# bioinformatics-ua/polus

Measured on AMD Instinct MI355X. Metric: train samples/sec BioBERT-base NER seq256, higher is better.
Workload: dtype bf16; 1 GPU; BERT-base (L=12,H=768,A=12,I=3072,V=28996) token classification C=4, seq_len=256, 64 samples/GPU, AdamW lr 5e-5 wd 0.01 warm-up 10%, dropout 0.1 (hidden + attention) (BASELINE.json configs[2] per-GPU shape), random-init weights; global_batch=64, seq_len=256, parallelism=dp1, grad_allreduce=none

## Files before the change

### polus_amd/csrc/common.h

```cpp
#pragma once
#include <hip/hip_runtime.h>
#include <stdint.h>
#include <stdio.h>
#include <string.h>
#include <math.h>

#include "../../include/polus_hip.h"

typedef __bf16 bf16_t;
typedef __bf16 bf16x8 __attribute__((ext_vector_type(8)));
typedef __bf16 bf16x4 __attribute__((ext_vector_type(4)));
typedef short s16x4 __attribute__((ext_vector_type(4)));
typedef float f32x4 __attribute__((ext_vector_type(4)));

void polus_set_error(const char* fmt, ...);
#define POLUS_FAIL(...) do { polus_set_error(__VA_ARGS__); return POLUS_ERR_INVALID; } while (0)
#define POLUS_REQUIRE(cond, ...) do { if (!(cond)) { polus_set_error(__VA_ARGS__); return POLUS_ERR_INVALID; } } while (0)
#define POLUS_CHECK_LAUNCH(name) do { hipError_t e__ = hipGetLastError(); \
    if (e__ != hipSuccess) { polus_set_error("%s: launch failed: %s", name, hipGetErrorString(e__)); return POLUS_ERR_HIP; } } while (0)
#define POLUS_HIP(call) do { hipError_t e__ = (call); \
    if (e__ != hipSuccess) { polus_set_error("%s failed: %s", #call, hipGetErrorString(e__)); return POLUS_ERR_HIP; } } while (0)

template <auto Kern, typename... A>
int polus_launch_lds(const char* who, dim3 grid, dim3 block, size_t lds_max, size_t lds, hipStream_t st, const A&... args) {
    static bool attr_done = false;
    if (!attr_done) {
        POLUS_HIP(hipFuncSetAttribute(reinterpret_cast<const void*>(Kern), hipFuncAttributeMaxDynamicSharedMemorySize, (int)lds_max));
        attr_done = true;
    }
    hipLaunchKernelGGL(Kern, grid, block, lds, st, args...);
    POLUS_CHECK_LAUNCH(who);
    return POLUS_OK;
}

static inline size_t polus_dtype_size(int dt) { return dt == POLUS_BF16 ? 2 : 4; }
static inline bool polus_aligned16(const void* p) { return (((uintptr_t)p) & 15) == 0; }

struct PolusCfg {
    int gemm_pp;
    int gemm_v1;
    int dw_ungrouped;
    int dw_fused_reduce;
    int ln_bwd_blocks;
    int ln_fin_single;
    int gemm_ring128;
    int gemm_auto_split;
    int ln_halfwave;
    int gemm_order;
    int gemm_persist;
    int reserve_cus;
    int attn_bwd_kres;
    int attn_debug;
    int dw_streamk;
    int dw_sk_cus;
    int dw_sk_delta;
    int attn_fused;
};
const PolusCfg& polus_cfg();
int polus_num_cus();
int polus_reserved_cus();

struct PolusDyn { uint32_t salt; float lr, lr_t; uint32_t pad; };
const PolusDyn* polus_dyn();
__device__ __forceinline__ uint32_t polus_eff_seed(uint32_t seed, const PolusDyn* dyn) {
    if (!dyn) return seed;
    uint32_t x = seed + dyn->salt;
    x ^= x >> 15;
    return x * 0x2C1B3C6Du;
}

template <typename T> __device__ __forceinline__ float to_f(T x);
template <> __device__ __forceinline__ float to_f<float>(float x) { return x; }
template <> __device__ __forceinline__ float to_f<bf16_t>(bf16_t x) { return (float)x; }
template <typename T> __device__ __forceinline__ T from_f(float x);
template <> __device__ __forceinline__ float from_f<float>(float x) { return x; }
template <> __device__ __forceinline__ bf16_t from_f<bf16_t>(float x) { return (bf16_t)x; }

template <typename T> __device__ __forceinline__ void load4(const T* p, float (&v)[4]);
template <> __device__ __forceinline__ void load4<float>(const float* p, float (&v)[4]) {
    float4 t = *reinterpret_cast<const float4*>(p); v[0] = t.x; v[1] = t.y; v[2] = t.z; v[3] = t.w;
}
template <> __device__ __forceinline__ void load4<bf16_t>(const bf16_t* p, float (&v)[4]) {
    bf16x4 t = *reinterpret_cast<const bf16x4*>(p);
    v[0] = (float)t[0]; v[1] = (float)t[1]; v[2] = (float)t[2]; v[3] = (float)t[3];
}
template <typename T> __device__ __forceinline__ void store4(T* p, const float (&v)[4]);
template <> __device__ __forceinline__ void store4<float>(float* p, const float (&v)[4]) {
    *reinterpret_cast<float4*>(p) = make_float4(v[0], v[1], v[2], v[3]);
}
template <> __device__ __forceinline__ void store4<bf16_t>(bf16_t* p, const float (&v)[4]) {
    bf16x4 t; t[0] = (bf16_t)v[0]; t[1] = (bf16_t)v[1]; t[2] = (bf16_t)v[2]; t[3] = (bf16_t)v[3];
    *reinterpret_cast<bf16x4*>(p) = t;
}

__device__ __forceinline__ float erf_fast(float x) {
    const float ax = fabsf(x);
    const float t = __frcp_rn(1.0f + 0.3275911f * ax);
    float poly = 1.061405429f;
    poly = poly * t - 1.453152027f;
    poly = poly * t + 1.421413741f;
    poly = poly * t - 0.284496736f;
    poly = poly * t + 0.254829592f;
    const float r = 1.0f - poly * t * __expf(-ax * ax);
    return copysignf(r, x);
}
__device__ __forceinline__ float gelu_f(float x) { return 0.5f * x * (1.0f + erf_fast(x * 0.70710678118654752f)); }
__device__ __forceinline__ float gelu_grad_f(float x) {
    float cdf = 0.5f * (1.0f + erf_fast(x * 0.70710678118654752f));
    float pdf = 0.3989422804014327f * __expf(-0.5f * x * x);
    return cdf + x * pdf;
}
__device__ __forceinline__ float swish_f(float x) { return x / (1.0f + __expf(-x)); }
__device__ __forceinline__ float swish_grad_f(float x) {
    float s = 1.0f / (1.0f + __expf(-x));
    return s * (1.0f + x * (1.0f - s));
}
typedef float f32x2_t __attribute__((ext_vector_type(2)));
__device__ __forceinline__ f32x2_t gelu_poly2(f32x2_t x, const float (&c)[11]) {
    f32x2_t xc = {__builtin_amdgcn_fmed3f(x[0], -4.5f, 4.5f), __builtin_amdgcn_fmed3f(x[1], -4.5f, 4.5f)};
    f32x2_t s = xc * xc;
    f32x2_t u = __builtin_elementwise_fma(s, (f32x2_t){2.0f / 20.25f, 2.0f / 20.25f}, (f32x2_t){-1.0f, -1.0f});
    f32x2_t r = {c[10], c[10]};
#pragma unroll
    for (int k = 9; k >= 0; --k) r = __builtin_elementwise_fma(r, u, (f32x2_t){c[k], c[k]});
    return __builtin_elementwise_fma(xc, r, (f32x2_t){0.5f, 0.5f});
}
__device__ __forceinline__ f32x2_t gelu_cdf2(f32x2_t x) {
    const float q[11] = {1.569049305e-01f, -7.719386095e-02f, 5.470119065e-02f, -4.010921159e-02f, 2.828393083e-02f,
                         -1.902094059e-02f, 1.143922652e-02f, -5.251548121e-03f, 2.716277400e-03f, -2.340015935e-03f,
                         9.806926012e-04f};
    return gelu_poly2(x, q);
}
__device__ __forceinline__ f32x2_t gelu_grad2(f32x2_t x) {
    const float w[11] = {1.594289755e-01f, -9.003904569e-02f, 8.714168751e-02f, -9.350841452e-02f, 9.645831298e-02f,
                         -9.557466143e-02f, 7.437658385e-02f, -3.356380937e-02f, 2.252388123e-02f, -3.068672777e-02f,
                         1.457471506e-02f};
    return gelu_poly2(x, w);
}
// ... 131 lines not shown
```

### polus_amd/csrc/norm.hip

```cpp
#include "common.h"

namespace {

constexpr int MAXC = 8;
constexpr int WAVES = 16;
constexpr int LN_THREADS = 64 * WAVES;
constexpr int MAX_PARTIAL_BLOCKS = 256;

__device__ __forceinline__ int n_chunks(int H) { return (H + 255) >> 8; }

template <typename T, int NC>
__device__ __forceinline__ void load_row(const T* row, int H, int lane, float (&v)[NC][4]) {
#pragma unroll
    for (int c = 0; c < NC; ++c) {
        int col = (lane + 64 * c) * 4;
        if (col < H) load4<T>(row + col, v[c]);
        else { v[c][0] = v[c][1] = v[c][2] = v[c][3] = 0.f; }
    }
}

template <int NC>
__device__ __forceinline__ void load_feat(const float* __restrict__ p, int H, int lane, float (&v)[NC][4]) {
#pragma unroll
    for (int c = 0; c < NC; ++c) {
// ... 192 lines not shown
        if (col < H) {
#pragma unroll
            for (int e = 0; e < 4; ++e) {
                xh[c][e] = (xv[c][e] - mu) * rs;
                dxh[c][e] = dy[c][e] * gv[c][e];
                s1 += dxh[c][e];
                s2 += dxh[c][e] * xh[c][e];
                acc.dg[c][e] += dy[c][e] * xh[c][e];
                acc.db[c][e] += dy[c][e];
            }
        } else {
#pragma unroll
            for (int e = 0; e < 4; ++e) xh[c][e] = dxh[c][e] = 0.f;
        }
    }
    s1 = wave_sum(s1) / (float)H;
    s2 = wave_sum(s2) / (float)H;
#pragma unroll
    for (int c = 0; c < NC; ++c) {
        int col = (lane + 64 * c) * 4;
        if (col < H) {
            float o[4], om[4];
#pragma unroll
            for (int e = 0; e < 4; ++e) { o[e] = (dxh[c][e] - s1 - xh[c][e] * s2) * rs; om[e] = o[e]; }
            if (out_drop.thresh) polus_dropout_run<4>(om, out_drop.seed, rowbase + col, out_drop.thresh, out_drop.inv, true);
            if (want_bias) {
#pragma unroll
                for (int e = 0; e < 4; ++e) acc.dbias[c][e] += om[e];
            }
            store4<TDX>(dxrow + col, o);
            if (dxm_row) store4<TDX>(dxm_row + col, om);
        }
    }
}

constexpr int BWD_WAVES = 4, BWD_MAX_BLOCKS = 1024, FIN_GROUP = 128;
template <typename T, int NC>
__global__ __launch_bounds__(64 * BWD_WAVES) void ln_bwd_kernel(const T* __restrict__ dy, const T* __restrict__ x,
                                                     const float* __restrict__ gamma, const float* __restrict__ mean,
                                                     const float* __restrict__ rstd, T* __restrict__ dx,
                                                     float* __restrict__ partial, int rows, int H, int want_bias,
                                                     T* __restrict__ dxm, DropArgs drop) {
    if (drop.thresh) drop.seed = polus_eff_seed(drop.seed, drop.dyn);
    extern __shared__ __attribute__((aligned(16))) unsigned char smem_raw[];
    float* lds = reinterpret_cast<float*>(smem_raw);
    const int lane = threadIdx.x & 63, wid = threadIdx.x >> 6;
    ColAcc<NC> acc;
    colacc_zero(acc);
    float gv[NC][4];
    load_feat<NC>(gamma, H, lane, gv);
    for (int row = blockIdx.x * BWD_WAVES + wid; row < rows; row += gridDim.x * BWD_WAVES) {
        float xv[NC][4];
        load_row<T, NC>(x + (long)row * H, H, lane, xv);
        ln_bwd_row<T, T, NC>(xv, dy + (long)row * H, gv, dx + (long)row * H, H, lane, mean[row], rstd[row], acc, want_bias,
                             dxm ? dxm + (long)row * H : nullptr, drop, DropArgs{0, 0, 1.f}, (unsigned)row * (unsigned)H);
    }
    colacc_flush_par<NC, BWD_WAVES>(acc, lds, partial, H, lane, wid, want_bias);
}

__global__ __launch_bounds__(1024) void colsum_finalize_kernel(const float* __restrict__ partial, int P, int pstride,
                                                               int ncols, int seg, float* out0, float* out1,
                                                               float* out2, int accumulate, int pgroup = 0) {
    __shared__ float red[16][64];
    const int cx = threadIdx.x & 63, gy = threadIdx.x >> 6;
    const int col = blockIdx.x * 64 + cx;
    float s = 0.f;
    if (pgroup > 0) {
        const int p0 = blockIdx.y * pgroup;
        partial += (long)p0 * pstride;
        P = min(pgroup, P - p0);
        out0 += (long)blockIdx.y * ncols;
    }
    if (col < ncols) {
#pragma unroll 8
        for (int p = gy; p < P; p += 16) s += partial[(long)p * pstride + col];
    }
    red[gy][cx] = s;
    __syncthreads();
    if (gy == 0 && col < ncols) {
        float t = 0.f;
#pragma unroll
        for (int k = 0; k < 16; ++k) t += red[k][cx];
        int which = col / seg, c = col % seg;
        float* out = which == 0 ? out0 : which == 1 ? out1 : out2;
        if (out) out[c] = accumulate ? out[c] + t : t;
    }
}

template <int NC>
__global__ __launch_bounds__(64 * BWD_WAVES) void ln_bwd_hw_kernel(const bf16_t* __restrict__ dy, const bf16_t* __restrict__ x,
                                                                    const float* __restrict__ gamma, const float* __restrict__ mean,
                                                                    const float* __restrict__ rstd, bf16_t* __restrict__ dx,
                                                                    float* __restrict__ partial, int rows, int H, int want_bias,
                                                                    bf16_t* __restrict__ dxm, DropArgs drop) {
    if (drop.thresh) drop.seed = polus_eff_seed(drop.seed, drop.dyn);
    extern __shared__ __attribute__((aligned(16))) unsigned char smem_raw[];
    float* lds = reinterpret_cast<float*>(smem_raw);
    const int lane = threadIdx.x & 63, wid = threadIdx.x >> 6, half = lane >> 5, hl = lane & 31;
    float gv[NC][8], adg[NC][8], adb[NC][8], abias[NC][8];
#pragma unroll
    for (int c = 0; c < NC; ++c) {
        const int col = (hl + 32 * c) * 8;
        load4<float>(gamma + col, *reinterpret_cast<float(*)[4]>(&gv[c][0])); load4<float>(gamma + col + 4, *reinterpret_cast<float(*)[4]>(&gv[c][4]));
#pragma unroll
        for (int e = 0; e < 8; ++e) adg[c][e] = adb[c][e] = abias[c][e] = 0.f;
    }
    const float invH = 1.0f / (float)H;
    for (int row = (blockIdx.x * BWD_WAVES + wid) * 2 + half; row < rows; row += gridDim.x * BWD_WAVES * 2) {
        const float mu = mean[row], rs = rstd[row];
        float xh[NC][8], dxh[NC][8];
        float s1 = 0.f, s2 = 0.f;
#pragma unroll
        for (int c = 0; c < NC; ++c) {
            const long off = (long)row * H + (hl + 32 * c) * 8;
            const bf16x8v tx = *reinterpret_cast<const bf16x8v*>(x + off);
            const bf16x8v td = *reinterpret_cast<const bf16x8v*>(dy + off);
#pragma unroll
            for (int e = 0; e < 8; ++e) {
                const float d = (float)td[e];
                xh[c][e] = ((float)tx[e] - mu) * rs;
                dxh[c][e] = d * gv[c][e];
                s1 += dxh[c][e];
                s2 += dxh[c][e] * xh[c][e];
                adg[c][e] += d * xh[c][e];
                adb[c][e] += d;
            }
        }
        s1 = half_sum(s1) * invH;
        s2 = half_sum(s2) * invH;
#pragma unroll
        for (int c = 0; c < NC; ++c) {
            const int col = (hl + 32 * c) * 8;
            float o[8], om[8];
#pragma unroll
            for (int e = 0; e < 8; ++e) { o[e] = (dxh[c][e] - s1 - xh[c][e] * s2) * rs; om[e] = o[e]; }
            if (drop.thresh) polus_dropout_run<8>(om, drop.seed, (unsigned)row * (unsigned)H + col, drop.thresh, drop.inv, true);
            if (want_bias) {
#pragma unroll
                for (int e = 0; e < 8; ++e) abias[c][e] += om[e];
            }
            bf16x8v t;
#pragma unroll
            for (int e = 0; e < 8; ++e) t[e] = (bf16_t)o[e];
            *reinterpret_cast<bf16x8v*>(dx + (long)row * H + col) = t;
            if (dxm) {
#pragma unroll
                for (int e = 0; e < 8; ++e) t[e] = (bf16_t)om[e];
                *reinterpret_cast<bf16x8v*>(dxm + (long)row * H + col) = t;
            }
        }
    }
    float* mine = lds + (long)wid * 3 * H;
#pragma unroll
    for (int c = 0; c < NC; ++c) {
        const int col = (hl + 32 * c) * 8;
#pragma unroll
        for (int e = 0; e < 8; ++e) {
            adg[c][e] += __shfl_xor(adg[c][e], 32, 64);
            adb[c][e] += __shfl_xor(adb[c][e], 32, 64);
            abias[c][e] += __shfl_xor(abias[c][e], 32, 64);
        }
        if (half == 0) {
            *reinterpret_cast<float4*>(mine + col) = make_float4(adg[c][0], adg[c][1], adg[c][2], adg[c][3]);
            *reinterpret_cast<float4*>(mine + col + 4) = make_float4(adg[c][4], adg[c][5], adg[c][6], adg[c][7]);
            *reinterpret_cast<float4*>(mine + H + col) = make_float4(adb[c][0], adb[c][1], adb[c][2], adb[c][3]);
            *reinterpret_cast<float4*>(mine + H + col + 4) = make_float4(adb[c][4], adb[c][5], adb[c][6], adb[c][7]);
            *reinterpret_cast<float4*>(mine + 2 * H + col) = make_float4(abias[c][0], abias[c][1], abias[c][2], abias[c][3]);
// ... 176 lines not shown
#pragma unroll
                for (int k = 0; k < 4; ++k)
                    row[j][c][k] = (valid && c * 256 + k * 64 + lane < H) ? src[c * 256 + k * 64] : 0.f;
        }
#pragma unroll
        for (int t = 0; t < SC_RUN; ++t) {
            const int id = __shfl(mine, t, 64);
            const unsigned same = (unsigned)__ballot(mine == id);
            if (id < 0 || (same & ((1u << t) - 1u))) continue;
            float* dst = gword + (long)id * H + lane;
#pragma unroll
            for (int c = 0; c < NC; ++c)
#pragma unroll
                for (int k = 0; k < 4; ++k) {
                    float acc = row[t][c][k];
#pragma unroll
                    for (int j = t + 1; j < SC_RUN; ++j)
                        if ((same >> j) & 1u) acc += row[j][c][k];
                    if (c * 256 + k * 64 + lane < H) atomicAdd(dst + c * 256 + k * 64, acc);
                }
        }
    }
}
__global__ __launch_bounds__(LN_THREADS) void embed_scatter_atomic_wide_kernel(const float* __restrict__ de, const int32_t* __restrict__ ids,
                                                                        float* __restrict__ gword, int rows, int H, int vocab) {
    const int lane = threadIdx.x & 63, wid = threadIdx.x >> 6;
    for (int row = blockIdx.x * WAVES + wid; row < rows; row += gridDim.x * WAVES) {
        int id = ids[row]; id = id < 0 ? 0 : (id >= vocab ? vocab - 1 : id);
        const float* src = de + (long)row * H;
        float* dst = gword + (long)id * H;
        for (int col = lane; col < H; col += 64) atomicAdd(dst + col, src[col]);
    }
}

__global__ __launch_bounds__(LN_THREADS) void embed_scatter_owner_kernel(const float* __restrict__ de, const int32_t* __restrict__ ids,
                                                                  float* __restrict__ gword, int rows, int H, int vocab) {
    const int lane = threadIdx.x & 63, wid = threadIdx.x >> 6;
    for (int row = blockIdx.x * WAVES + wid; row < rows; row += gridDim.x * WAVES) {
        auto clampid = [vocab](int v) { return v < 0 ? 0 : (v >= vocab ? vocab - 1 : v); };
        const int cid = clampid(ids[row]);
        bool dup = false;
        for (int j0 = 0; j0 < row && !dup; j0 += 64) {
            int j = j0 + lane;
            bool hit = (j < row) && (clampid(ids[j]) == cid);
            dup = __any(hit);
        }
        if (dup) continue;
        float* dst = gword + (long)cid * H;
        for (int c0 = 0; c0 < H; c0 += 64 * 4) {
            int col = c0 + lane * 4;
            float a[4] = {0.f, 0.f, 0.f, 0.f};
            for (int j0 = row; j0 < rows; j0 += 64) {
                int j = j0 + lane;
                unsigned long long m = __ballot((j < rows) && (clampid(ids[j]) == cid));
                while (m) {
                    int b = __ffsll((long long)m) - 1;
                    m &= m - 1;
                    if (col < H) {
                        float v[4];
                        load4<float>(de + (long)(j0 + b) * H + col, v);
#pragma unroll
                        for (int e = 0; e < 4; ++e) a[e] += v[e];
                    }
                }
            }
            if (col < H) {
                float o[4];
                load4<float>(dst + col, o);
#pragma unroll
                for (int e = 0; e < 4; ++e) o[e] += a[e];
                store4<float>(dst + col, o);
            }
        }
    }
}

__global__ __launch_bounds__(256) void embed_pos_grad_kernel(const float* __restrict__ de, float* __restrict__ gpos,
                                                             int B, int S, int H, int accumulate) {
    long idx = (long)blockIdx.x * blockDim.x + threadIdx.x;
    if (idx >= (long)S * H) return;
    float s = 0.f;
    for (int b = 0; b < B; ++b) s += de[(long)b * S * H + idx];
    gpos[idx] = accumulate ? gpos[idx] + s : s;
}

}

extern "C" size_t polus_layernorm_bwd_workspace_bytes(int rows, int H) {
    int b = ln_bwd_blocks(rows), b2 = ln_blocks(rows);
    if (b2 > b) b = b2;
    int groups = (b + FIN_GROUP - 1) / FIN_GROUP;
    return ((size_t)b + groups) * 3 * (size_t)H * sizeof(float);
}

extern "C" int polus_layernorm_fwd(int dtype, const void* x, const float* gamma, const float* beta,
                                   void* y, float* mean, float* rstd, int rows, int H, float eps, void* stream) {
    POLUS_REQUIRE(x && gamma && beta && y && mean && rstd, "polus_layernorm_fwd: null pointer");
    POLUS_REQUIRE(rows > 0 && H > 0 && H % 4 == 0 && H <= 256 * MAXC, "polus_layernorm_fwd: H=%d must be a multiple of 4, <= %d", H, 256 * MAXC);
    POLUS_REQUIRE(polus_aligned16(x) && polus_aligned16(y) && polus_aligned16(gamma) && polus_aligned16(beta),
                  "polus_layernorm_fwd: pointers must be 16-byte aligned");
    hipStream_t st = static_cast<hipStream_t>(stream);
    int blocks = (rows + WAVES - 1) / WAVES;
    if (blocks > 4096) blocks = 4096;
    if (dtype == POLUS_BF16 && H % 256 == 0 && H <= 1024 && rows % 2 == 0 && polus_cfg().ln_halfwave) {
        const int fw = 4;
        int hb = (rows / 2 + fw - 1) / fw;
        if (hb > 16384) hb = 16384;
        const int LN_THREADS_HW = 64 * fw;
        if (H == 256) hipLaunchKernelGGL(ln_fwd_hw_kernel<1>, dim3(hb), dim3(LN_THREADS_HW), 0, st, (const bf16_t*)x, gamma, beta, (bf16_t*)y, mean, rstd, rows, H, eps);
        else if (H == 512) hipLaunchKernelGGL(ln_fwd_hw_kernel<2>, dim3(hb), dim3(LN_THREADS_HW), 0, st, (const bf16_t*)x, gamma, beta, (bf16_t*)y, mean, rstd, rows, H, eps);
        else if (H == 768) hipLaunchKernelGGL(ln_fwd_hw_kernel<3>, dim3(hb), dim3(LN_THREADS_HW), 0, st, (const bf16_t*)x, gamma, beta, (bf16_t*)y, mean, rstd, rows, H, eps);
        else hipLaunchKernelGGL(ln_fwd_hw_kernel<4>, dim3(hb), dim3(LN_THREADS_HW), 0, st, (const bf16_t*)x, gamma, beta, (bf16_t*)y, mean, rstd, rows, H, eps);
    } else if (dtype == POLUS_BF16)
        POLUS_NC_DISPATCH(H, bf16_t, ln_fwd_kernel, dim3(blocks), dim3(LN_THREADS), 0, st, (const bf16_t*)x, gamma, beta, (bf16_t*)y, mean, rstd, rows, H, eps);
    else if (dtype == POLUS_F32)
        POLUS_NC_DISPATCH(H, float, ln_fwd_kernel, dim3(blocks), dim3(LN_THREADS), 0, st, (const float*)x, gamma, beta, (float*)y, mean, rstd, rows, H, eps);
    else POLUS_FAIL("polus_layernorm_fwd: bad dtype");
    POLUS_CHECK_LAUNCH("polus_layernorm_fwd");
    return POLUS_OK;
}

extern "C" int polus_layernorm_bwd(int dtype, const void* dy, const void* x, const float* gamma,
                                   const float* mean, const float* rstd, void* dx,
                                   float* dgamma, float* dbeta, float* dbias, int accumulate,
                                   int rows, int H, void* dx_masked, float drop_p, uint32_t seed,
                                   void* workspace, size_t workspace_bytes, void* stream) {
    const bool defer = !dgamma && !dbeta;
    POLUS_REQUIRE(dy && x && gamma && mean && rstd && dx && (defer || (dgamma && dbeta)), "polus_layernorm_bwd: null pointer");
    POLUS_REQUIRE(drop_p >= 0.f && drop_p < 1.f && (long)rows * H < (1LL << 32), "polus_layernorm_bwd: bad dropout arguments");
    POLUS_REQUIRE(!(drop_p > 0.f) || dx_masked, "polus_layernorm_bwd: dropout needs dx_masked");
    DropArgs drop{drop_p > 0.f ? polus_drop_thresh(drop_p) : 0u, seed, 1.0f / (1.0f - drop_p), polus_dyn()};
    POLUS_REQUIRE(rows > 0 && H > 0 && H % 4 == 0 && H <= 256 * MAXC, "polus_layernorm_bwd: bad H=%d", H);
    POLUS_REQUIRE(polus_aligned16(x) && polus_aligned16(dy) && polus_aligned16(dx) && polus_aligned16(gamma),
                  "polus_layernorm_bwd: pointers must be 16-byte aligned");
    size_t need = polus_layernorm_bwd_workspace_bytes(rows, H);
    if (!workspace || workspace_bytes < need) { polus_set_error("polus_layernorm_bwd: workspace %zu < %zu", workspace_bytes, need); return POLUS_ERR_WORKSPACE; }
    hipStream_t st = static_cast<hipStream_t>(stream);
    int blocks = ln_bwd_blocks(rows);
    float* partial = static_cast<float*>(workspace);
    size_t lds = (size_t)BWD_WAVES * 3 * (size_t)H * sizeof(float);
    int wb = dbias ? 1 : 0;
    if (dtype == POLUS_BF16 && H % 256 == 0 && H <= 1024 && rows % 2 == 0 && polus_cfg().ln_halfwave && polus_aligned16(dx_masked)) {
#define POLUS_LN_BWD_HW(NCV) hipLaunchKernelGGL(ln_bwd_hw_kernel<NCV>, dim3(blocks), dim3(64 * BWD_WAVES), lds, st, (const bf16_t*)dy, (const bf16_t*)x, gamma, mean, rstd, (bf16_t*)dx, partial, rows, H, wb, (bf16_t*)dx_masked, drop)
        if (H == 256) POLUS_LN_BWD_HW(1); else if (H == 512) POLUS_LN_BWD_HW(2); else if (H == 768) POLUS_LN_BWD_HW(3); else POLUS_LN_BWD_HW(4);
#undef POLUS_LN_BWD_HW
    } else if (dtype == POLUS_BF16)
        POLUS_NC_DISPATCH(H, bf16_t, ln_bwd_kernel, dim3(blocks), dim3(64 * BWD_WAVES), lds, st, (const bf16_t*)dy, (const bf16_t*)x, gamma, mean, rstd, (bf16_t*)dx, partial, rows, H, wb, (bf16_t*)dx_masked, drop);
    else if (dtype == POLUS_F32)
        POLUS_NC_DISPATCH(H, float, ln_bwd_kernel, dim3(blocks), dim3(64 * BWD_WAVES), lds, st, (const float*)dy, (const float*)x, gamma, mean, rstd, (float*)dx, partial, rows, H, wb, (float*)dx_masked, drop);
    else POLUS_FAIL("polus_layernorm_bwd: bad dtype");
    POLUS_CHECK_LAUNCH("polus_layernorm_bwd");
    if (defer) return POLUS_OK;
    int ncols = (wb ? 3 : 2) * H;
    if (blocks > polus_cfg().ln_fin_single) {
        int groups = (blocks + FIN_GROUP - 1) / FIN_GROUP;
        float* part2 = partial + (size_t)blocks * 3 * H;
        hipLaunchKernelGGL(colsum_finalize_kernel, dim3((ncols + 63) / 64, groups), dim3(1024), 0, st,
                           partial, blocks, 3 * H, ncols, ncols, part2, (float*)nullptr, (float*)nullptr, 0, FIN_GROUP);
        POLUS_CHECK_LAUNCH("polus_layernorm_bwd(finalize 1)");
        hipLaunchKernelGGL(colsum_finalize_kernel, dim3((ncols + 63) / 64), dim3(1024), 0, st,
                           part2, groups, ncols, ncols, H, dgamma, dbeta, dbias, accumulate, 0);
    } else {
        hipLaunchKernelGGL(colsum_finalize_kernel, dim3((ncols + 63) / 64), dim3(1024), 0, st,
                           partial, blocks, 3 * H, ncols, H, dgamma, dbeta, dbias, accumulate, 0);
    }
    POLUS_CHECK_LAUNCH("polus_layernorm_bwd(finalize)");
    return POLUS_OK;
}

extern "C" int polus_layernorm_bwd_finalize(void* workspace, size_t workspace_bytes, int rows, int H, float* dgamma, float* dbeta,
                                            float* dbias, int accumulate, void* stream) {
    POLUS_REQUIRE(workspace && dgamma && dbeta && rows > 0 && H > 0 && H % 4 == 0, "polus_layernorm_bwd_finalize: bad arguments");
    size_t need = polus_layernorm_bwd_workspace_bytes(rows, H);
    if (workspace_bytes < need) { polus_set_error("polus_layernorm_bwd_finalize: workspace %zu < %zu", workspace_bytes, need); return POLUS_ERR_WORKSPACE; }
    hipStream_t st = static_cast<hipStream_t>(stream);
    const int blocks = ln_bwd_blocks(rows);
    float* partial = static_cast<float*>(workspace);
    const int ncols = (dbias ? 3 : 2) * H;
    if (blocks > polus_cfg().ln_fin_single) {
        int groups = (blocks + FIN_GROUP - 1) / FIN_GROUP;
        float* part2 = partial + (size_t)blocks * 3 * H;
        hipLaunchKernelGGL(colsum_finalize_kernel, dim3((ncols + 63) / 64, groups), dim3(1024), 0, st,
                           partial, blocks, 3 * H, ncols, ncols, part2, (float*)nullptr, (float*)nullptr, 0, FIN_GROUP);
        POLUS_CHECK_LAUNCH("polus_layernorm_bwd_finalize(1)");
        hipLaunchKernelGGL(colsum_finalize_kernel, dim3((ncols + 63) / 64), dim3(1024), 0, st,
                           part2, groups, ncols, ncols, H, dgamma, dbeta, dbias, accumulate, 0);
    } else {
        hipLaunchKernelGGL(colsum_finalize_kernel, dim3((ncols + 63) / 64), dim3(1024), 0, st,
                           partial, blocks, 3 * H, ncols, H, dgamma, dbeta, dbias, accumulate, 0);
    }
    POLUS_CHECK_LAUNCH("polus_layernorm_bwd_finalize");
    return POLUS_OK;
}

extern "C" size_t polus_colsum_workspace_bytes(int rows, int cols) {
    int chunks = (rows + 63) / 64;
    if (chunks > 256) chunks = 256;
    if (chunks < 1) chunks = 1;
    return (size_t)chunks * (size_t)cols * sizeof(float);
}

extern "C" int polus_colsum(int dtype, const void* x, long ldx, int rows, int cols, float* out, int accumulate,
                            void* workspace, size_t workspace_bytes, void* stream) {
    POLUS_REQUIRE(x && out && rows > 0 && cols > 0 && ldx >= cols, "polus_colsum: bad arguments");
    POLUS_REQUIRE(dtype == POLUS_F32 || dtype == POLUS_BF16, "polus_colsum: bad dtype");
    return colsum_launch(dtype, x, ldx, rows, cols, out, accumulate, nullptr, 0, workspace, workspace_bytes,
                         static_cast<hipStream_t>(stream));
}

extern "C" size_t polus_embed_bwd_workspace_bytes(int B, int S, int H) {
    size_t rows = (size_t)B * S;
    size_t de = rows * H * sizeof(float);
    size_t part = polus_layernorm_bwd_workspace_bytes((int)rows, H);
    size_t cs = polus_colsum_workspace_bytes((int)rows, H);
    return de + (part > cs ? part : cs) + 256;
}

extern "C" int polus_embed_ln_fwd(int dtype, const int32_t* ids, const int32_t* type_ids,
                                  const float* word, const float* pos, const float* type,
                                  const float* gamma, const float* beta, void* y, float* mean, float* rstd,
                                  int B, int S, int H, int vocab, int max_pos, int type_vocab, float eps,
                                  float drop_p, uint32_t seed, void* stream) {
    POLUS_REQUIRE(ids && word && pos && type && gamma && beta && y && mean && rstd, "polus_embed_ln_fwd: null pointer");
    POLUS_REQUIRE(drop_p >= 0.f && drop_p < 1.f, "polus_embed_ln_fwd: bad drop_p");
    const unsigned dthresh = drop_p > 0.f ? polus_drop_thresh(drop_p) : 0u;
    const float dinv = 1.0f / (1.0f - drop_p);
    POLUS_REQUIRE(B > 0 && S > 0 && S <= max_pos, "polus_embed_ln_fwd: S=%d exceeds max_position_embeddings=%d", S, max_pos);
    POLUS_REQUIRE(H % 4 == 0 && H <= 256 * MAXC && vocab > 0 && type_vocab > 0, "polus_embed_ln_fwd: bad H=%d", H);
    POLUS_REQUIRE(polus_aligned16(word) && polus_aligned16(pos) && polus_aligned16(type) && polus_aligned16(y) &&
                  polus_aligned16(gamma) && polus_aligned16(beta), "polus_embed_ln_fwd: pointers must be 16-byte aligned");
    hipStream_t st = static_cast<hipStream_t>(stream);
    int rows = B * S, blocks = (rows + WAVES - 1) / WAVES;
    if (blocks > 4096) blocks = 4096;
    if (dtype == POLUS_BF16)
        POLUS_NC_DISPATCH(H, bf16_t, embed_fwd_kernel, dim3(blocks), dim3(LN_THREADS), 0, st, ids, type_ids, word, pos, type, gamma, beta, (bf16_t*)y, mean, rstd, B, S, H, vocab, type_vocab, eps, dthresh, seed, dinv, polus_dyn());
    else if (dtype == POLUS_F32)
        POLUS_NC_DISPATCH(H, float, embed_fwd_kernel, dim3(blocks), dim3(LN_THREADS), 0, st, ids, type_ids, word, pos, type, gamma, beta, (float*)y, mean, rstd, B, S, H, vocab, type_vocab, eps, dthresh, seed, dinv, polus_dyn());
    else POLUS_FAIL("polus_embed_ln_fwd: bad dtype");
    POLUS_CHECK_LAUNCH("polus_embed_ln_fwd");
    return POLUS_OK;
}

extern "C" int polus_embed_ln_bwd(int dtype, const void* dy, const int32_t* ids, const int32_t* type_ids,
                                  const float* word, const float* pos, const float* type, const float* gamma,
                                  const float* mean, const float* rstd,
                                  float* gword, float* gpos, float* gtype, float* ggamma, float* gbeta,
                                  int accumulate, int deterministic,
                                  int B, int S, int H, int vocab, int max_pos, int type_vocab,
                                  float drop_p, uint32_t seed,
                                  void* workspace, size_t workspace_bytes, void* stream) {
    DropArgs in_drop{drop_p > 0.f ? polus_drop_thresh(drop_p) : 0u, seed, 1.0f / (1.0f - drop_p), polus_dyn()};
    POLUS_REQUIRE(dy && ids && word && pos && type && gamma && mean && rstd && gword && gpos && gtype && ggamma && gbeta,
                  "polus_embed_ln_bwd: null pointer");
    POLUS_REQUIRE(B > 0 && S > 0 && S <= max_pos && H % 4 == 0 && H <= 256 * MAXC, "polus_embed_ln_bwd: bad shape");
    POLUS_REQUIRE(polus_aligned16(dy) && polus_aligned16(gword) && polus_aligned16(workspace),
                  "polus_embed_ln_bwd: pointers must be 16-byte aligned");
    size_t need = polus_embed_bwd_workspace_bytes(B, S, H);
    if (!workspace || workspace_bytes < need) { polus_set_error("polus_embed_ln_bwd: workspace %zu < %zu", workspace_bytes, need); return POLUS_ERR_WORKSPACE; }
    hipStream_t st = static_cast<hipStream_t>(stream);
    const int rows = B * S;
    float* de = static_cast<float*>(workspace);
    size_t de_bytes = ((size_t)rows * H * sizeof(float) + 255) / 256 * 256;
    float* partial = reinterpret_cast<float*>(static_cast<unsigned char*>(workspace) + de_bytes);
    size_t partial_bytes = workspace_bytes - de_bytes;
    int blocks = ln_blocks(rows);
    size_t lds = 3 * (size_t)H * sizeof(float);
    if (dtype == POLUS_BF16)
        POLUS_NC_DISPATCH(H, bf16_t, embed_bwd_ln_kernel, dim3(blocks), dim3(LN_THREADS), lds, st, (const bf16_t*)dy, ids, type_ids, word, pos, type, gamma, mean, rstd, de, partial, B, S, H, vocab, type_vocab, in_drop);
    else if (dtype == POLUS_F32)
        POLUS_NC_DISPATCH(H, float, embed_bwd_ln_kernel, dim3(blocks), dim3(LN_THREADS), lds, st, (const float*)dy, ids, type_ids, word, pos, type, gamma, mean, rstd, de, partial, B, S, H, vocab, type_vocab, in_drop);
    else POLUS_FAIL("polus_embed_ln_bwd: bad dtype");
    POLUS_CHECK_LAUNCH("polus_embed_ln_bwd(ln)");
    hipLaunchKernelGGL(colsum_finalize_kernel, dim3((2 * H + 63) / 64), dim3(1024), 0, st,
                       partial, blocks, 3 * H, 2 * H, H, ggamma, gbeta, (float*)nullptr, accumulate);
    POLUS_CHECK_LAUNCH("polus_embed_ln_bwd(finalize)");

    if (!accumulate) {
        POLUS_HIP(hipMemsetAsync(gword, 0, (size_t)vocab * H * sizeof(float), st));
        POLUS_HIP(hipMemsetAsync(gpos, 0, (size_t)max_pos * H * sizeof(float), st));
    }
    int sblocks = (rows + WAVES - 1) / WAVES;
    if (sblocks > 4096) sblocks = 4096;
    if (deterministic)
        hipLaunchKernelGGL(embed_scatter_owner_kernel, dim3(sblocks), dim3(LN_THREADS), 0, st, de, ids, gword, rows, H, vocab);
    else
    {
        const dim3 g(min((rows + SC_RUN * SC_WAVES - 1) / (SC_RUN * SC_WAVES), 4096)), b(64 * SC_WAVES);
        if (H <= 256) hipLaunchKernelGGL(embed_scatter_atomic_kernel<1>, g, b, 0, st, de, ids, gword, rows, H, vocab);
        else if (H <= 512) hipLaunchKernelGGL(embed_scatter_atomic_kernel<2>, g, b, 0, st, de, ids, gword, rows, H, vocab);
        else if (H <= 768) hipLaunchKernelGGL(embed_scatter_atomic_kernel<3>, g, b, 0, st, de, ids, gword, rows, H, vocab);
        else if (H <= 1024) hipLaunchKernelGGL(embed_scatter_atomic_kernel<4>, g, b, 0, st, de, ids, gword, rows, H, vocab);
        else hipLaunchKernelGGL(embed_scatter_atomic_wide_kernel, dim3(sblocks), dim3(LN_THREADS), 0, st, de, ids, gword, rows, H, vocab);
    }
    POLUS_CHECK_LAUNCH("polus_embed_ln_bwd(scatter)");
    hipLaunchKernelGGL(embed_pos_grad_kernel, dim3(((long)S * H + 255) / 256), dim3(256), 0, st, de, gpos, B, S, H, accumulate);
    POLUS_CHECK_LAUNCH("polus_embed_ln_bwd(pos)");
    for (int t = 0; t < type_vocab; ++t) {
        if (type_ids) {
            int rc = colsum_launch(POLUS_F32, de, H, rows, H, gtype + (long)t * H, accumulate, type_ids, t, partial, partial_bytes, st);
            if (rc != POLUS_OK) return rc;
        } else if (t == 0) {
            int rc = colsum_launch(POLUS_F32, de, H, rows, H, gtype, accumulate, nullptr, 0, partial, partial_bytes, st);
            if (rc != POLUS_OK) return rc;
        } else if (!accumulate) {
            POLUS_HIP(hipMemsetAsync(gtype + (long)t * H, 0, (size_t)H * sizeof(float), st));
        }
    }
    return POLUS_OK;
}
```

### polus_amd/csrc/runtime.hip

```cpp
#include "common.h"
#include <stdarg.h>

static thread_local char g_err[512] = "";

void polus_set_error(const char* fmt, ...) {
    va_list ap;
    va_start(ap, fmt);
    vsnprintf(g_err, sizeof(g_err), fmt, ap);
    va_end(ap);
}

extern "C" const char* polus_last_error(void) { return g_err; }

static PolusCfg g_cfg;
static bool g_cfg_ready = false;
static int env_int(const char* name, int dflt) {
    const char* e = getenv(name);
    return (e && *e) ? atoi(e) : dflt;
}
static void read_cfg() {
    g_cfg.gemm_pp = env_int("POLUS_GEMM_PP", 0);
    g_cfg.gemm_v1 = getenv("POLUS_GEMM_V1") != nullptr;
    g_cfg.dw_ungrouped = getenv("POLUS_DW_UNGROUPED") != nullptr;
    g_cfg.gemm_order = env_int("POLUS_GEMM_ORDER", 4);
    g_cfg.reserve_cus = env_int("POLUS_GEMM_RESERVE_CUS", 0);
    g_cfg.gemm_persist = env_int("POLUS_GEMM_PERSIST", 1);
    g_cfg.dw_fused_reduce = env_int("POLUS_DW_FUSED_REDUCE", 1);
    g_cfg.attn_fused = env_int("POLUS_ATTN_FUSED", 1);
    g_cfg.attn_bwd_kres = env_int("POLUS_ATTN_BWD_KRES", 1);
    g_cfg.attn_debug = env_int("POLUS_ATTN_DEBUG", 0);
    g_cfg.ln_halfwave = env_int("POLUS_LN_HALFWAVE", 1);
    g_cfg.gemm_auto_split = env_int("POLUS_GEMM_AUTO_SPLIT", 1);
    g_cfg.gemm_ring128 = env_int("POLUS_GEMM_RING128", 0);
    g_cfg.ln_bwd_blocks = env_int("POLUS_LN_BWD_BLOCKS", 512);
    g_cfg.ln_fin_single = env_int("POLUS_LN_FIN_SINGLE", 512);
    g_cfg.dw_streamk = env_int("POLUS_DW_STREAMK", 0);
    g_cfg.dw_sk_delta = env_int("POLUS_DW_SK_DELTA", 2);
    g_cfg.dw_sk_cus = env_int("POLUS_DW_SK_CUS", 0);
    g_cfg_ready = true;
}
const PolusCfg& polus_cfg() {
    if (!g_cfg_ready) read_cfg();
    return g_cfg;
}
extern "C" int polus_reload_env(void) { read_cfg(); return POLUS_OK; }

int polus_num_cus() {
    static int n = 0;
    if (!n) {
        int dev = 0; hipDeviceProp_t prop;
        if (hipGetDevice(&dev) == hipSuccess && hipGetDeviceProperties(&prop, dev) == hipSuccess) n = prop.multiProcessorCount;
        if (n <= 0) n = 256;
    }
    return n;
}
static int g_reserve_on = 1;
extern "C" int polus_set_reserve_active(int on) { g_reserve_on = on != 0; return POLUS_OK; }
int polus_reserved_cus() { return g_reserve_on ? polus_cfg().reserve_cus : 0; }

static const PolusDyn* g_dyn = nullptr;
const PolusDyn* polus_dyn() { return g_dyn; }
extern "C" int polus_set_dynamic_params(const void* dev_block16) {
    POLUS_REQUIRE(dev_block16 == nullptr || polus_aligned16(dev_block16), "polus_set_dynamic_params: the block must be 16-byte aligned");
    g_dyn = static_cast<const PolusDyn*>(dev_block16);
    return POLUS_OK;
}
extern "C" int polus_abi_version(void) { return POLUS_ABI_VERSION; }

extern "C" int polus_device_info(int* n_cu, int* lds_bytes_per_cu, char* arch, int arch_len) {
    int dev = 0;
    POLUS_HIP(hipGetDevice(&dev));
    hipDeviceProp_t prop;
    POLUS_HIP(hipGetDeviceProperties(&prop, dev));
    if (n_cu) *n_cu = prop.multiProcessorCount;
    if (lds_bytes_per_cu) *lds_bytes_per_cu = (int)prop.maxSharedMemoryPerMultiProcessor;
    if (arch && arch_len > 0) {
        strncpy(arch, prop.gcnArchName, arch_len - 1);
        arch[arch_len - 1] = 0;
    }
    return POLUS_OK;
}

namespace {

template <typename S, typename D>
__global__ void cast_kernel(const S* __restrict__ src, D* __restrict__ dst, int64_t n) {
    int64_t i4 = ((int64_t)blockIdx.x * blockDim.x + threadIdx.x) * 4;
    const int64_t stride = (int64_t)gridDim.x * blockDim.x * 4;
    for (; i4 < n; i4 += stride) {
        if (i4 + 4 <= n) {
            float v[4];
            load4<S>(src + i4, v);
            store4<D>(dst + i4, v);
        } else {
            for (int64_t j = i4; j < n; ++j) dst[j] = from_f<D>(to_f<S>(src[j]));
        }
    }
}

__global__ void scale_kernel(float* __restrict__ x, float a, int64_t n) {
    int64_t i4 = ((int64_t)blockIdx.x * blockDim.x + threadIdx.x) * 4;
    const int64_t stride = (int64_t)gridDim.x * blockDim.x * 4;
    for (; i4 < n; i4 += stride) {
        if (i4 + 4 <= n) {
            float4 v = *reinterpret_cast<float4*>(x + i4);
            v.x *= a; v.y *= a; v.z *= a; v.w *= a;
            *reinterpret_cast<float4*>(x + i4) = v;
        } else {
            for (int64_t j = i4; j < n; ++j) x[j] *= a;
        }
    }
}

template <typename T>
// ... 195 lines not shown
```

Baseline: 5412 samples/s.

## Fuse embedding LayerNorm backward with word, position and type gradient scatter

Adds a one-pass embedding backward kernel, one block per sequence position. It computes the LayerNorm backward for the B rows at that position, accumulates the position and token-type gradients in registers and LDS, and scatters word gradients with atomics after merging duplicate ids inside a wave. This replaces the staged path, which wrote an fp32 dx buffer of size rows*H and then ran separate position, type and word reduction kernels. The fused path is on by default, is skipped in deterministic mode, and depends on float atomics into gword, so summation order and bitwise results are no longer fixed. It only supports up to 4 token types, and the 256 blocks may leave the GPU underused.

```diff
diff --git a/polus_amd/csrc/common.h b/polus_amd/csrc/common.h
--- a/polus_amd/csrc/common.h
+++ b/polus_amd/csrc/common.h
@@ -54,6 +54,7 @@
     int dw_streamk;
     int dw_sk_cus;
     int dw_sk_delta;
+    int embed_fused;
     int attn_fused;
 };
 const PolusCfg& polus_cfg();
diff --git a/polus_amd/csrc/norm.hip b/polus_amd/csrc/norm.hip
--- a/polus_amd/csrc/norm.hip
+++ b/polus_amd/csrc/norm.hip
@@ -298,7 +298,7 @@
 #pragma unroll
         for (int k = 0; k < 16; ++k) t += red[k][cx];
         int which = col / seg, c = col % seg;
-        float* out = which == 0 ? out0 : which == 1 ? out1 : out2;
+        float* out = which == 0 ? out0 : which == 1 ? out1 : (out2 ? out2 + (long)(which - 2) * seg : nullptr);
         if (out) out[c] = accumulate ? out[c] + t : t;
     }
 }
@@ -641,6 +641,112 @@
     float s = 0.f;
     for (int b = 0; b < B; ++b) s += de[(long)b * S * H + idx];
     gpos[idx] = accumulate ? gpos[idx] + s : s;
+}
+
+template <int NC> struct EmbFused { static constexpr int W = NC <= 3 ? 16 : (NC == 4 ? 8 : 4); };
+constexpr int EMB_FUSED_MAX_TYPES = 4;
+
+template <typename T, int NC>
+__global__ __launch_bounds__(64 * EmbFused<NC>::W) void embed_bwd_fused_kernel(
+        const T* __restrict__ dy, const int32_t* __restrict__ ids, const int32_t* __restrict__ tts,
+        const float* __restrict__ word, const float* __restrict__ pos, const float* __restrict__ type,
+        const float* __restrict__ gamma, const float* __restrict__ mean, const float* __restrict__ rstd,
+        float* __restrict__ gword, float* __restrict__ gpos, float* __restrict__ partial,
+        int B, int S, int H, int vocab, int type_vocab, int accumulate, DropArgs in_drop) {
+    constexpr int W = EmbFused<NC>::W, THREADS = 64 * W;
+    constexpr int PC = (NC * 256 + THREADS - 1) / THREADS;
+    if (in_drop.thresh) in_drop.seed = polus_eff_seed(in_drop.seed, in_drop.dyn);
+    extern __shared__ __attribute__((aligned(16))) unsigned char smem_raw[];
+    float* rowbuf = reinterpret_cast<float*>(smem_raw);
+    float* tacc = rowbuf + (long)W * H;
+    const int lane = threadIdx.x & 63, wid = threadIdx.x >> 6, tid = threadIdx.x;
+    const int s = blockIdx.x;
+    for (int idx = tid; idx < type_vocab * H; idx += THREADS) tacc[idx] = 0.f;
+    ColAcc<NC> acc;
+    colacc_zero(acc);
+    float gv[NC][4];
+    load_feat<NC>(gamma, H, lane, gv);
+    float pacc[PC];
+#pragma unroll
+    for (int k = 0; k < PC; ++k) pacc[k] = 0.f;
+    float* myrow = rowbuf + (long)wid * H;
+    for (int b0 = 0; b0 < B; b0 += W) {
+        int mine = -1, mytt = 0;
+        if (lane < W && b0 + lane < B) {
+            const long r = (long)(b0 + lane) * S + s;
+            mine = ids[r]; mine = mine < 0 ? 0 : (mine >= vocab ? vocab - 1 : mine);
+            mytt = tts ? tts[r] : 0; mytt = mytt < 0 ? 0 : (mytt >= type_vocab ? type_vocab - 1 : mytt);
+        }
+        const int id = __shfl(mine, wid, 64), tt = __shfl(mytt, wid, 64);
+        if (id >= 0) {
+            const int row = (b0 + wid) * S + s;
+            float xv[NC][4];
+            gather_sum<T, NC>(word, pos, type, id, s, tt, H, lane, xv);
+            ln_bwd_row<T, float, NC>(xv, dy + (long)row * H, gv, myrow, H, lane, mean[row], rstd[row], acc, 0,
+                                     nullptr, DropArgs{0, 0, 1.f}, in_drop, (unsigned)row * (unsigned)H);
+        }
+        __syncthreads();
+        const int nrows = min(W, B - b0);
+        for (int w = 0; w < nrows; ++w) {
+            float* trow = tacc + (long)__shfl(mytt, w, 64) * H;
+#pragma unroll
+            for (int k = 0; k < PC; ++k) {
+                const int col = tid + k * THREADS;
+                if (col < H) {
+                    const float v = rowbuf[(long)w * H + col];
+                    pacc[k] += v;
+                    trow[col] += v;
+                }
+            }
+        }
+        for (int w = 0; w < nrows; ++w) {
+            const int wid_id = __shfl(mine, w, 64);
+            const unsigned same = (unsigned)__ballot(mine == wid_id);
+            if (same & ((1u << w) - 1u)) continue;
+            float* dst = gword + (long)wid_id * H;
+#pragma unroll
+            for (int k = 0; k < PC; ++k) {
+                const int col = tid + k * THREADS;
+                if (col < H) {
+                    float a = rowbuf[(long)w * H + col];
+                    for (unsigned rest = same >> (w + 1) << (w + 1); rest; rest &= rest - 1)
+                        a += rowbuf[(long)(__ffs(rest) - 1) * H + col];
+                    atomicAdd(dst + col, a);
+                }
+            }
+        }
+        __syncthreads();
+    }
+    float* dst = partial + (long)blockIdx.x * (2 + type_vocab) * H;
+#pragma unroll
+    for (int k = 0; k < PC; ++k) {
+        const int col = tid + k * THREADS;
+        if (col < H) {
+            const long i = (long)s * H + col;
+            gpos[i] = accumulate ? gpos[i] + pacc[k] : pacc[k];
+            for (int t = 0; t < type_vocab; ++t) dst[(long)(2 + t) * H + col] = tacc[(long)t * H + col];
+        }
+    }
+#pragma unroll
+    for (int which = 0; which < 2; ++which) {
+#pragma unroll
+        for (int c = 0; c < NC; ++c) {
+            const int col = (lane + 64 * c) * 4;
+            if (col < H) store4<float>(myrow + col, which == 0 ? acc.dg[c] : acc.db[c]);
+        }
+        __syncthreads();
+#pragma unroll
+        for (int k = 0; k < PC; ++k) {
+            const int col = tid + k * THREADS;
+            if (col < H) {
+                float t = rowbuf[col];
+#pragma unroll
+                for (int w = 1; w < W; ++w) t += rowbuf[(long)w * H + col];
+                dst[(long)which * H + col] = t;
+            }
+        }
+        __syncthreads();
+    }
 }
 
 }
@@ -772,7 +878,9 @@
     size_t de = rows * H * sizeof(float);
     size_t part = polus_layernorm_bwd_workspace_bytes((int)rows, H);
     size_t cs = polus_colsum_workspace_bytes((int)rows, H);
-    return de + (part > cs ? part : cs) + 256;
+    size_t staged = de + (part > cs ? part : cs) + 256;
+    size_t fused = (size_t)S * (2 + EMB_FUSED_MAX_TYPES) * H * sizeof(float);
+    return staged > fused ? staged : fused;
 }
 
 extern "C" int polus_embed_ln_fwd(int dtype, const int32_t* ids, const int32_t* type_ids,
@@ -818,6 +926,28 @@
     if (!workspace || workspace_bytes < need) { polus_set_error("polus_embed_ln_bwd: workspace %zu < %zu", workspace_bytes, need); return POLUS_ERR_WORKSPACE; }
     hipStream_t st = static_cast<hipStream_t>(stream);
     const int rows = B * S;
+    if (!deterministic && polus_cfg().embed_fused) {
+        POLUS_REQUIRE(type_vocab > 0 && type_vocab <= EMB_FUSED_MAX_TYPES, "polus_embed_ln_bwd: type_vocab=%d, the one-pass path takes up to %d (POLUS_EMBED_FUSED=0 for the staged one)", type_vocab, EMB_FUSED_MAX_TYPES);
+        const int nc = (H + 255) / 256, W = nc <= 3 ? 16 : (nc == 4 ? 8 : 4);
+        const size_t lds = (size_t)(W + type_vocab) * H * sizeof(float);
+        POLUS_REQUIRE(lds <= 65536, "polus_embed_ln_bwd: H=%d with type_vocab=%d needs %zu bytes of LDS", H, type_vocab, lds);
+        if (!accumulate) {
+            POLUS_HIP(hipMemsetAsync(gword, 0, (size_t)vocab * H * sizeof(float), st));
+            if (max_pos > S) POLUS_HIP(hipMemsetAsync(gpos + (size_t)S * H, 0, (size_t)(max_pos - S) * H * sizeof(float), st));
+        }
+        float* partial = static_cast<float*>(workspace);
+        if (dtype == POLUS_BF16)
+            POLUS_NC_DISPATCH(H, bf16_t, embed_bwd_fused_kernel, dim3(S), dim3(64 * W), lds, st, (const bf16_t*)dy, ids, type_ids, word, pos, type, gamma, mean, rstd, gword, gpos, partial, B, S, H, vocab, type_vocab, accumulate, in_drop);
+        else if (dtype == POLUS_F32)
+            POLUS_NC_DISPATCH(H, float, embed_bwd_fused_kernel, dim3(S), dim3(64 * W), lds, st, (const float*)dy, ids, type_ids, word, pos, type, gamma, mean, rstd, gword, gpos, partial, B, S, H, vocab, type_vocab, accumulate, in_drop);
+        else POLUS_FAIL("polus_embed_ln_bwd: bad dtype");
+        POLUS_CHECK_LAUNCH("polus_embed_ln_bwd(fused)");
+        const int ncols = (2 + type_vocab) * H;
+        hipLaunchKernelGGL(colsum_finalize_kernel, dim3((ncols + 63) / 64), dim3(1024), 0, st,
+                           partial, S, ncols, ncols, H, ggamma, gbeta, gtype, accumulate);
+        POLUS_CHECK_LAUNCH("polus_embed_ln_bwd(finalize)");
+        return POLUS_OK;
+    }
     float* de = static_cast<float*>(workspace);
     size_t de_bytes = ((size_t)rows * H * sizeof(float) + 255) / 256 * 256;
     float* partial = reinterpret_cast<float*>(static_cast<unsigned char*>(workspace) + de_bytes);
diff --git a/polus_amd/csrc/runtime.hip b/polus_amd/csrc/runtime.hip
--- a/polus_amd/csrc/runtime.hip
+++ b/polus_amd/csrc/runtime.hip
@@ -30,6 +30,7 @@
     g_cfg.attn_bwd_kres = env_int("POLUS_ATTN_BWD_KRES", 1);
     g_cfg.attn_debug = env_int("POLUS_ATTN_DEBUG", 0);
     g_cfg.ln_halfwave = env_int("POLUS_LN_HALFWAVE", 1);
+    g_cfg.embed_fused = env_int("POLUS_EMBED_FUSED", 1);
     g_cfg.gemm_auto_split = env_int("POLUS_GEMM_AUTO_SPLIT", 1);
     g_cfg.gemm_ring128 = env_int("POLUS_GEMM_RING128", 0);
     g_cfg.ln_bwd_blocks = env_int("POLUS_LN_BWD_BLOCKS", 512);
```

Result: no change. 5447 samples/s, median of 6 (+0.6%).
